# CUAI/Edge-Proposal-Sets

Measured on AMD Instinct MI355X. Metric: candidate edges scored/sec on ogbl-ppa (ppa-like synthetic): Adamic-Adar over the FULL 2-hop non-edge candidate set + top-4M selection, higher is better.
Workload: dtype int64

## Files before the change

### edge-proposal-sets_amd/csrc/scan_pieces.hip

```cpp
#include "eps_common.h"
#include "scan_common.h"
#include <string.h>

#define SP_EMPTY 0u
#define SP_MAXP (SP_M + 1)
#define SP_UBITS 8192
#define SP_SB 4
#define SP_PACKED_X8 8u
#define SP_MODE_RATIO 2270u
#define SP_MODE_RATIO_WIDE 8000u
#define SP_BATCH 8
#define SP_EM 128
#define SP_G 1

typedef int sp_v4i __attribute__((ext_vector_type(4)));

struct sp_params {
    const int64_t *rowptr;
    const int32_t *col;
    const int32_t *revpos;
    const uint32_t *fx32;
    const float *val;
    const float *node_w;
    float up;
// ... 6 lines not shown
    uint32_t col_bytes;
    int32_t table_bits;
    uint32_t piece_paths;
    const uint32_t *ssum;
    const uint32_t *smax;
    uint32_t packed_paths;
    int32_t packed_dmax;
    const uint32_t *pptr;
    const uint4 *plan;
    uint32_t mode_ratio;
    int32_t shift;
    float scale;
    unsigned int *next_col;
    eps_survivors *out;
    unsigned int *status;
    const uint4 *colrec;
    const uint32_t *rowrec;
    uint32_t wide_paths;
    int32_t wide_rows;
    uint32_t sketch;
    uint32_t batch_from;
    const uint4 *pack;
    const uint2 *heads;
};

__device__ __forceinline__ void sp_barrier() { asm volatile("s_waitcnt lgkmcnt(0)\n\ts_barrier" ::: "memory"); }

__device__ __forceinline__ int sp_wave_incl_scan(int x)
{
    x += __builtin_amdgcn_update_dpp(0, x, 0x111, 0xF, 0xF, false);
    x += __builtin_amdgcn_update_dpp(0, x, 0x112, 0xF, 0xF, false);
    x += __builtin_amdgcn_update_dpp(0, x, 0x114, 0xF, 0xF, false);
    x += __builtin_amdgcn_update_dpp(0, x, 0x118, 0xF, 0xF, false);
    x += __builtin_amdgcn_update_dpp(0, x, 0x142, 0xA, 0xF, false);
    x += __builtin_amdgcn_update_dpp(0, x, 0x143, 0xC, 0xF, false);
    return x;
}

__device__ __forceinline__ uint32_t sp_wave_sum(uint32_t x)
{
    return (uint32_t)__builtin_amdgcn_readlane(sp_wave_incl_scan((int)x), 63);
}

typedef float sp_v4f __attribute__((ext_vector_type(4)));
typedef short sp_v2s __attribute__((ext_vector_type(2)));

__device__ __forceinline__ uint32_t sp_mix(uint32_t x) { return x * 0x9E3779B1u; }
__device__ __forceinline__ uint32_t sp_mix2(uint32_t x) { return x * 0x85EBCA6Bu; }

struct sp_unit {
    sp_v4i u4;
    sp_v4f a4;
    uint32_t fx;
    int nvalid;
};

template <class Emit>
__device__ __forceinline__ int sp_plan_column(const sp_params &p, int32_t v, int32_t dv, int lane, int32_t my_bound, uint32_t pwk,
                                              int32_t nbk, uint32_t direct_ids, Emit emit)
{
    const uint32_t ek = (uint32_t)sp_wave_incl_scan((int)pwk) - pwk;
    const bool pk_on = p.ssum != nullptr;
    const uint32_t sv = pk_on ? p.ssum[v] - (p.heads ? (p.heads[v].y < p.ssum[v] ? p.heads[v].y : p.ssum[v]) : 0u) : 0u;
    const uint32_t smk = pk_on ? p.smax[lane <= SP_M ? lane : SP_M] : 0u;
    const int kv = __popcll(__ballot(lane >= 1 && lane < SP_M && my_bound <= v - 1));
    const int32_t hi_k = my_bound < v ? my_bound : v;
    int np = 0, k0 = 0;
    while (k0 <= kv) {
        const int32_t lo = __builtin_amdgcn_readlane(my_bound, k0);
        const uint32_t e0 = (uint32_t)__builtin_amdgcn_readlane((int)ek, k0);
        const bool in = lane > k0 && lane <= kv + 1;
// ... 66 lines not shown
template <int T, bool HV, bool FULL, bool PACK, bool SK = false>
__global__ __launch_bounds__(T, 4) void scan_piece_kernel(sp_params p)
{
    extern __shared__ __attribute__((aligned(16))) uint32_t lds[];
    const int slots = 1 << p.table_bits;
    uint32_t *tkey = lds;
    uint32_t *tval = lds + slots;
    uint4 *r_desc = (uint4 *)(lds + 2 * slots);
    uint32_t *ubits = lds + ((2 * slots + 4 * (T + 1) + 3) & ~3);
    uint16_t *wrank = (uint16_t *)(ubits + SP_UBITS / 32);
    __shared__ unsigned long long s_alloc;
    __shared__ int s_rbase;
    __shared__ int32_t s_pk0[SP_MAXP], s_pk1[SP_MAXP];
    __shared__ int32_t s_plo[SP_MAXP], s_phi[SP_MAXP];
    __shared__ uint32_t s_pinfo[SP_MAXP];
    __shared__ uint32_t s_pq[SP_MAXP];
    __shared__ int32_t s_pna[SP_MAXP], s_pnb[SP_MAXP];
    __shared__ int s_np;
    __shared__ unsigned int s_ticket;
    __shared__ unsigned int s_out_cur, s_out_end;
    __shared__ unsigned int s_fill_lo, s_fill_hi;
    __shared__ unsigned int s_hot;
    __shared__ uint32_t s_em[SP_EM];

    const int tid = threadIdx.x, lane = tid & 63;
    const int wib = __builtin_amdgcn_readfirstlane(tid >> 6);
    const uint32_t out_cap = p.out->capacity;
    int64_t *__restrict__ out_key = p.out->key;
    float *__restrict__ out_val = p.out->val;
    const uint32_t *__restrict__ rowptr_lo = (const uint32_t *)p.rowptr;
    const __amdgpu_buffer_rsrc_t col_rs = __builtin_amdgcn_make_buffer_rsrc((void *)p.col, 0, p.col_bytes, 0x00020000);
    const __amdgpu_buffer_rsrc_t val_rs = __builtin_amdgcn_make_buffer_rsrc((void *)(HV ? (const void *)p.val : (const void *)p.col), 0,
                                                                            p.col_bytes, 0x00020000);
    const uint32_t thr32 = sp_bar_units(p.out->threshold, p.shift);
    const uint32_t direct_ids = 2u * (uint32_t)slots;
    const bool no_bar = !FULL && thr32 <= 1u;
    const bool raw_sums = FULL || p.heads != nullptr;
    const uint32_t chunk = no_bar && direct_ids > 8192u ? direct_ids : 8192u;
    const int32_t my_bound = p.bounds[lane <= SP_M ? lane : SP_M];

    for (int i = tid; i < 2 * slots; i += T) lds[i] = 0u;
    for (int i = tid; i < SP_UBITS / 32; i += T) ubits[i] = 0u;
    for (int i = tid; i < SP_EM; i += T) s_em[i] = 0u;
    if (tid == 0) {
        s_out_cur = 0u;
        s_out_end = 0u;
        s_fill_lo = 0u;
        s_fill_hi = 0u;
        s_alloc = 0ull;
    }
    bool sketch_seen = false;
    unsigned long long n_cand = 0;
    uint32_t new_keys = 0u;
    const unsigned int ncol = (unsigned int)p.n_columns;
    const unsigned int batch_from = p.batch_from;
    auto first_of = [&](unsigned int tk) { return tk < batch_from ? tk : batch_from + (tk - batch_from) * SP_BATCH; };
    unsigned int t = blockIdx.x < batch_from ? blockIdx.x : first_of(blockIdx.x);
    unsigned int t_end = t + (blockIdx.x < batch_from ? 1u : SP_BATCH);
    sp_barrier();

    while (t < ncol) {
        const bool last_of_ticket = t + 1u >= t_end || t + 1u >= ncol;
        unsigned int t_next = 0;
        if (tid == 0 && last_of_ticket) t_next = gridDim.x + atomicAdd(p.next_col, 1u);
        int32_t v, dv;
        uint32_t vb;
        uint4 cra = make_uint4(0u, 0u, 0u, 0u), crb = make_uint4(0u, 0u, 0u, 0u);
        if (FULL || p.colrec) {
            cra = p.colrec[2 * (size_t)t];
            crb = p.colrec[2 * (size_t)t + 1];
            v = (int32_t)cra.x;
            vb = cra.y;
            dv = (int32_t)cra.z;
        } else {
            v = p.columns[t];
            vb = rowptr_lo[2 * (size_t)v];
            dv = (int32_t)(rowptr_lo[2 * (size_t)v + 2] - vb);
        }
        const int32_t *__restrict__ vcol = p.col + vb;
        const int32_t *__restrict__ vrev = p.revpos + vb;
        const int rounds = (dv + T - 1) / T;
        const bool single = rounds == 1;
        uint32_t xv = 0u, thr_v = thr32;
        bool bad_head = false;
        if (FULL || p.heads) {
            const uint2 hd = (FULL || p.colrec) ? make_uint2(cra.w, crb.x) : p.heads[v];
            xv = hd.x;
            if (thr32 < SP_FLAG) {
                bad_head = hd.y >= thr32;
                thr_v = thr32 - hd.y;
            }
            if (bad_head && tid == 0) atomicOr(p.status, 4u);
            if ((FULL || p.ssum) && thr32 < SP_FLAG && ((FULL || p.colrec) ? crb.y : p.ssum[v]) < thr32) bad_head = true;
        }
        if (dv > 0 && v > 0 && !bad_head) {
            uint32_t my_w = 0, my_rev = 0, my_base = 0, my_fx = 0;
            uint32_t cut_first = 0u;
            if (PACK && single && tid < dv) {
                const uint4 pa = p.pack[2 * ((size_t)vb + (size_t)tid)];
                my_w = pa.x;
                my_base = pa.y;
                my_fx = pa.z;
                my_rev = pa.w & 0xFFFFu;
                cut_first = pa.w >> 16;
            }
            if (!PACK && single && tid < dv) {
                my_w = (uint32_t)vcol[tid];
                my_rev = (uint32_t)vrev[tid];
            }
            if (!PACK && single && tid < dv) {
                my_base = (FULL || p.rowrec) ? p.rowrec[(size_t)my_w * 32 + 16] : rowptr_lo[2 * (size_t)my_w];
                my_fx = HV ? __builtin_bit_cast(uint32_t, (p.val[vb + tid] * p.node_w[my_w]) * p.up)
                           : ((FULL || p.rowrec) ? p.rowrec[(size_t)my_w * 32 + 17] : p.fx32[my_w]);
            }
            if (!FULL && wib == 0 && !p.plan) {
                const uint32_t pwk = lane < SP_M ? p.wpaths[(size_t)v * SP_M + lane] : 0u;
                const int32_t nbk = lane >= 1 && lane <= SP_M ? (int32_t)p.cuts[(size_t)v * SP_M + lane - 1] : 0;
                const int np = sp_plan_column(p, v, dv, lane, my_bound, pwk, nbk, direct_ids,
                                              [&](int i, int k0, int k1, int32_t lo, int32_t hi, uint32_t info, uint32_t pq, int32_t na, int32_t nb) {
                                                  if (lane == 0) {
                                                      s_pk0[i] = k0;
                                                      s_pk1[i] = k1;
                                                      s_plo[i] = lo;
                                                      s_phi[i] = hi;
                                                      s_pinfo[i] = info;
                                                      s_pq[i] = pq;
                                                      s_pna[i] = na;
                                                      s_pnb[i] = nb;
                                                  }
                                              });
                if (lane == 0) s_np = np;
            } else if (FULL || p.plan) {
                const uint32_t pb = (FULL || p.colrec) ? crb.z : p.pptr[v];
                const int np = (FULL || p.colrec) ? (int)crb.w : (int)(p.pptr[v + 1] - pb);
                if (tid < np) {
                    const uint4 rec = p.plan[pb + (uint32_t)tid];
                    const int k1 = (int)((rec.y >> 8) & 0xFFu);
                    const int32_t bk = p.bounds[k1];
                    s_pinfo[tid] = rec.x;
                    s_pk0[tid] = (int)(rec.y & 0xFFu);
                    s_pk1[tid] = k1;
                    s_pq[tid] = rec.y >> 16;
                    s_pna[tid] = (int32_t)(rec.z & 0xFFFFu);
                    s_pnb[tid] = (int32_t)(rec.z >> 16);
                    s_plo[tid] = (int32_t)rec.w;
                    s_phi[tid] = bk < v ? bk : v;
                }
                if (tid == 0) s_np = np;
            }
            sp_barrier();
            const int np = s_np;
            uint32_t cut_ahead = 0u, seg_from = 0u;
            const uint16_t *__restrict__ cut_tab = (FULL || p.rowrec) ? (const uint16_t *)p.rowrec : p.cuts;
            const size_t cut_ld = (FULL || p.rowrec) ? 64u : (size_t)SP_M;
// ... 34 lines not shown
                const uint32_t mask = (1u << bits) - 1u;
                const uint32_t span = (uint32_t)(hi_id - lo_id);
                const uint32_t scan_slots = d16 ? (span + 1u) >> 1 : direct ? span : (1u << bits);
                const uint32_t cand_max = direct ? span : (1u << bits);
                if (tid == 0) {
                    s_hot = 0u;
                    uint32_t need = ppaths < cand_max ? ppaths : cand_max;
                    if (!no_bar && need > 1024u) need = 1024u;
                    if (need > chunk) need = chunk;
                    const uint32_t left = s_out_cur < s_out_end ? s_out_end - s_out_cur : 0u;
                    if (left < need) {
                        s_fill_lo = s_out_cur < out_cap ? s_out_cur : out_cap;
                        s_fill_hi = left ? (s_out_end < out_cap ? s_out_end : out_cap) : s_fill_lo;
                        const unsigned long long b64 = atomicAdd(&p.out->count, (unsigned long long)chunk);
                        const uint32_t b = b64 < (unsigned long long)out_cap ? (uint32_t)b64 : out_cap;
                        s_out_cur = b;
                        s_out_end = b + chunk;
                    }
                }
                uint32_t seg_a = 0u, seg_len = 0u;
                if (single && tid < dv) {
                    const uint32_t b = cut_ahead < my_rev ? cut_ahead : my_rev;
                    seg_a = seg_from;
                    seg_len = (uint32_t)tid < xv ? 0u : b - seg_from;
                    seg_from = b;
                    if (pi + 1 < np)
                        cut_ahead = PACK && pi + 1 <= 8 ? pack16[((size_t)vb + (size_t)tid) * 16 + 7 + (pi + 1)]
                                                        : cut_tab[(size_t)my_w * cut_ld + s_pk1[pi + 1] - 1];
                }
                auto emit = [&](uint32_t u, uint32_t sum) {
                    uint32_t pos = atomicAdd(&s_out_cur, 1u);
                    if (pos >= s_out_end) {
                        const unsigned long long q = atomicAdd(&p.out->count, 1ull);
                        pos = q < (unsigned long long)out_cap ? (uint32_t)q : out_cap;
                    }
                    if (pos < out_cap) {
                        out_key[pos] = ((int64_t)v << 32) | (int64_t)u;
                        out_val[pos] = raw_sums ? __builtin_bit_cast(float, sum) : (float)sum * p.scale;
                    }
                };
                for (uint32_t part = 0; part < parts; ++part) {
                    for (int j = sketch ? nb : single ? tid : na + tid; j < nb; j += T) {
                        const uint32_t u = single ? my_w : (uint32_t)vcol[j];
                        if (j >= na && (int32_t)u >= lo_id && (int32_t)u < hi_id) {
                            if (d16) {
                                const uint32_t o = u - (uint32_t)lo_id;
                                atomicOr(&lds[o >> 1], 0x8000u << ((o & 1u) << 4));
                            } else if (direct) {
                                lds[u - (uint32_t)lo_id] = SP_FLAG;
                            } else if (packed) {
                                const uint32_t mix = sp_mix(u);
                                uint32_t h = mix >> (32 - bits);
                                const uint32_t st = ((mix >> 7) | 1u) & mask;
                                const uint32_t word = ((u - (uint32_t)lo_id) << pk_sb) | pk_flag;
                                for (uint32_t tries = 0; tries <= mask; ++tries) {
                                    if (atomicCAS(&lds[h], 0u, word) == 0u) break;
                                    h = (h + st) & mask;
                                }
                            } else {
                                const uint32_t mix = sp_mix(u);
                                if ((mix & (parts - 1u)) == part) {
                                    uint32_t h = mix >> (32 - bits);
                                    const uint32_t st = ((mix >> 7) | 1u) & mask;
// ... 91 lines not shown
                            for (int q = 0; q < SP_G; ++q) {
                                const int s = (int)ulo + (it0 + q) * T + tid;
                                const uint4 rd = r_desc[lo[q]];
                                const uint32_t us = rd.w, rl = rd.y, rs = rd.x;
                                f[q].fx = rd.z;
                                const bool in = s < (int)uhi;
                                const int off = (s - (int)us) * 4;
                                int left = (int)rl - off;
                                left = in ? left : 0;
                                f[q].nvalid = left < 0 ? 0 : (left > 4 ? 4 : left);
                                const uint32_t at = in ? rs + (uint32_t)off : (p.col_bytes >> 2);
                                f[q].u4 = __builtin_amdgcn_raw_buffer_load_b128(col_rs, (int)(at * 4u), 0, 0);
                                if (HV) f[q].a4 = __builtin_bit_cast(sp_v4f, __builtin_amdgcn_raw_buffer_load_b128(val_rs, (int)(at * 4u), 0, 0));
                            }
                        };
                        auto path_fx = [&](const sp_unit &f, int e) -> uint32_t {
                            if (!HV) return f.fx;
                            return (uint32_t)__builtin_ceilf(f.a4[e] * __builtin_bit_cast(float, f.fx)) + 1u;
                        };
                        auto consume_group = [&](const sp_unit (&f)[SP_G]) {
                            if (sketch) {
                                const uint32_t half = 1u << (bits - 1);
#pragma unroll
                                for (int q = 0; q < SP_G; ++q)
#pragma unroll
                                    for (int e = 0; e < 4; ++e)
                                        if (e < f[q].nvalid) {
                                            const uint32_t id = (uint32_t)f[q].u4[e];
                                            atomicAdd(&lds[sp_mix(id) >> (33 - bits)], f[q].fx);
                                            atomicAdd(&lds[half + (sp_mix2(id) >> (33 - bits))], f[q].fx);
                                        }
                            } else if (d16) {
#pragma unroll
                                for (int q = 0; q < SP_G; ++q)
#pragma unroll
                                    for (int e = 0; e < 4; ++e)
                                        if (e < f[q].nvalid) {
                                            const uint32_t o = (uint32_t)(f[q].u4[e] - lo_id);
                                            atomicAdd(&lds[o >> 1], f[q].fx << ((o & 1u) << 4));
                                        }
                            } else if (direct) {
#pragma unroll
                                for (int q = 0; q < SP_G; ++q)
#pragma unroll
                                    for (int e = 0; e < 4; ++e)
                                        if (e < f[q].nvalid) atomicAdd(&lds[(uint32_t)(f[q].u4[e] - lo_id)], path_fx(f[q], e));
                            } else if (packed) {
                                constexpr int E = 4 * SP_G;
                                uint32_t lid[E], h[E], mixv[E], old[E];
                                uint32_t pend = 0u;
#pragma unroll
                                for (int q = 0; q < SP_G; ++q) pend |= ((1u << f[q].nvalid) - 1u) << (4 * q);
#pragma unroll
                                for (int i = 0; i < E; ++i) {
// ... 126 lines not shown
                                        have = false;
                                        pend = 0u;
                                    }
                                }
                            }
                        };
                        {
                            const int n_iter = (int)(uhi - ulo + T - 1) / T;
                            sp_unit fa[SP_G], fb[SP_G];
                            fetch_group(0, fa);
                            if (n_iter <= SP_G) {
                                consume_group(fa);
                            } else {
                                for (int it0 = 0; it0 < n_iter; it0 += 2 * SP_G) {
                                    fetch_group(it0 + SP_G, fb);
                                    consume_group(fa);
                                    fetch_group(it0 + 2 * SP_G, fa);
                                    consume_group(fb);
                                }
                            }
                        }
                        if (sketch) {
                            if (tid == 0 && !sketch_seen) atomicOr(p.status, 16u);
                            sketch_seen = true;
                            sp_barrier();
                            const uint32_t half = 1u << (bits - 1);
                            {
                                uint32_t mx = 0u;
                                for (uint32_t i = 4u * (uint32_t)tid; i < half; i += 4u * T) {
                                    const uint4 a4 = *(const uint4 *)(lds + i);
                                    const uint32_t m01 = a4.x > a4.y ? a4.x : a4.y, m23 = a4.z > a4.w ? a4.z : a4.w;
                                    const uint32_t m = m01 > m23 ? m01 : m23;
                                    mx = m > mx ? m : mx;
                                }
                                if (__ballot(mx >= thr_v) && lane == 0) s_hot = 1u;
                            }
                            sp_barrier();
                            if (s_hot) {
                            const int n_iter = (int)(uhi - ulo + T - 1) / T;
                            auto report = [&](uint32_t u, uint32_t est) {
                                int a = na, b = nb;
                                while (a < b) {
                                    const int mid = (a + b) >> 1;
                                    if (vcol[mid] < (int32_t)u) a = mid + 1; else b = mid;
                                }
                                if (a < nb && vcol[a] == (int32_t)u) return;
                                const uint32_t em_mask = (p.sketch >> 1 ? p.sketch >> 1 : (uint32_t)SP_EM) - 1u;
                                uint32_t h = (sp_mix(u) >> 9) & em_mask;
                                for (uint32_t tries = 0; tries <= em_mask; ++tries) {
                                    const uint32_t old = atomicCAS(&s_em[h], 0u, u + 1u);
                                    if (old == 0u) {
                                        emit(u, est);
                                        return;
                                    }
                                    if (old == u + 1u) return;
                                    h = (h + 1u) & em_mask;
                                }
                                atomicOr(p.status, 8u);
                            };
                            auto look = [&](const sp_unit (&f)[SP_G]) {
                                uint32_t est[4 * SP_G];
#pragma unroll
                                for (int i = 0; i < 4 * SP_G; ++i) {
                                    const uint32_t id = (uint32_t)f[i >> 2].u4[i & 3];
                                    const uint32_t ea = lds[sp_mix(id) >> (33 - bits)], eb = lds[half + (sp_mix2(id) >> (33 - bits))];
                                    est[i] = ea < eb ? ea : eb;
                                }
#pragma unroll
                                for (int i = 0; i < 4 * SP_G; ++i)
                                    if ((i & 3) < f[i >> 2].nvalid && est[i] >= thr_v) report((uint32_t)f[i >> 2].u4[i & 3], est[i]);
                            };
                            sp_unit fa[SP_G], fb[SP_G];
                            fetch_group(0, fa);
                            if (n_iter <= SP_G) {
                                look(fa);
                            } else {
                                for (int it0 = 0; it0 < n_iter; it0 += 2 * SP_G) {
                                    fetch_group(it0 + SP_G, fb);
                                    look(fa);
                                    fetch_group(it0 + 2 * SP_G, fa);
                                    look(fb);
                                }
                            }
                            }
                        }
                            if (uhi < (uint32_t)total) sp_barrier();
                        }
                        sp_barrier();
                        for (int i = tid; i < SP_UBITS / 32; i += T) ubits[i] = 0u;
                        if (tid == 0) {
                            s_alloc = 0ull;
                            s_fill_hi = 0u;
                        }
// ... 97 lines not shown
                            for (int b = 0; b < SP_SB; ++b) {
                                const uint32_t i = i0 + 4u * T * b + 4u * tid;
                                const int sv[4] = {(int)s4[b].x, (int)s4[b].y, (int)s4[b].z, (int)s4[b].w};
                                const int m01 = sv[0] > sv[1] ? sv[0] : sv[1], m23 = sv[2] > sv[3] ? sv[2] : sv[3];
                                if ((m01 > m23 ? m01 : m23) >= thr_s) {
#pragma unroll
                                    for (int e = 0; e < 4; ++e)
                                        if (sv[e] >= thr_s) emit(tkey[i + e] - 1u, (uint32_t)sv[e]);
                                }
                                if (i < scan_slots) {
                                    *(uint4 *)(tkey + i) = make_uint4(0u, 0u, 0u, 0u);
                                    *(uint4 *)(tval + i) = make_uint4(0u, 0u, 0u, 0u);
                                }
                            }
                        }
                    }
                    n_cand += (unsigned long long)cnt_here + (unsigned long long)new_keys;
                    new_keys = 0u;
                    sp_barrier();
                }
            }
        }
        if (!last_of_ticket) {
            ++t;
            sp_barrier();
            continue;
        }
        if (tid == 0) s_ticket = t_next;
        sp_barrier();
        const unsigned int tk = s_ticket;
        sp_barrier();
        t = first_of(tk);
        t_end = t + (tk < batch_from ? 1u : SP_BATCH);
    }
    {
        const uint32_t f0 = s_out_cur < out_cap ? s_out_cur : out_cap, f1 = s_out_end < out_cap ? s_out_end : out_cap;
        for (uint32_t i = f0 + (uint32_t)tid; i < f1; i += T) {
            out_key[i] = -1;
            out_val[i] = -__builtin_inff();
        }
    }
    {
        unsigned long long x = n_cand;
#pragma unroll
        for (int d = 32; d >= 1; d >>= 1) x += __shfl_xor(x, d);
        if (lane == 0 && x) atomicAdd(&p.out->n_candidates, x);
    }
// ... 616 lines not shown
    EPS_REQUIRE((ssum_or_null == nullptr) == (smax_or_null == nullptr), "eps_scan_screen: ssum and smax come together");
    EPS_REQUIRE(!heads_or_null || plan_or_null, "eps_scan_screen: a head table comes with the plan table built for it");
    return sp_launch(rowptr, col, nullptr, revpos, fx32, nullptr, cuts, wpaths, ssum_or_null, smax_or_null, pptr_or_null,
                     plan_or_null, heads_or_null, rowrec_or_null, pack_or_null, bounds, n_nodes, nnz, columns, colrec_or_null, n_columns,
                     batch_from, shift, variant, out, status, stream);
}

extern "C" int eps_scan_screen_weighted(const int64_t *rowptr, const int32_t *col, const float *val, const int32_t *revpos,
                                        const float *node_w, const uint16_t *cuts, const uint32_t *wpaths,
                                        const int32_t *bounds, int64_t n_nodes, int64_t nnz, const int32_t *columns,
                                        int64_t n_columns, int32_t shift, int32_t variant, eps_survivors *out, uint32_t *status,
                                        void *stream)
{
    EPS_REQUIRE(n_columns == 0 || n_nodes == 0 || (val && node_w), "eps_scan_screen_weighted: null pointer");
    return sp_launch(rowptr, col, val, revpos, nullptr, node_w, cuts, wpaths, nullptr, nullptr, nullptr, nullptr, nullptr, nullptr, nullptr,
                     bounds, n_nodes, nnz, columns, nullptr, n_columns, n_columns, shift, variant, out, status, stream);
}

static const int sp_threads_of[3] = {512, 1024, 256}, sp_bits_of[3] = {13, 14, 12}, sp_per_cu[3] = {2, 1, 4};
#define SP_VARIANT_GEOM(v) ((v) & 0xFF)
#define SP_VARIANT_DMAX(v) ((((v) >> 8) & 0xFF) - 1)
#define SP_VARIANT_WIDE(v) (((v) >> 24) & 1)
#define SP_VARIANT_SKETCH(v) (((v) >> 16) & 0xFF)

static void sp_plan_geometry(sp_params &p, const uint16_t *cuts, const uint32_t *wpaths, const uint32_t *ssum, const uint32_t *smax,
                             const int32_t *bounds, int64_t n_nodes, int32_t shift, int32_t variant, int32_t dmax_arg)
{
    const int bits = sp_bits_of[variant];
    p.cuts = cuts;
    p.wpaths = wpaths;
    p.bounds = bounds;
    p.n_nodes = (int32_t)n_nodes;
    p.table_bits = bits;
    p.piece_paths = (1u << bits) / 2u;
    p.ssum = ssum;
    p.smax = smax;
    p.packed_paths = (SP_PACKED_X8 << bits) / 8u;
    p.packed_dmax = shift > 8 ? (shift - 8 < 24 ? shift - 8 : 24) : 0;
    if (dmax_arg >= 0 && dmax_arg < p.packed_dmax) p.packed_dmax = dmax_arg;
    p.mode_ratio = SP_MODE_RATIO;
    p.shift = shift;
}

__global__ __launch_bounds__(256) void sp_plan_kernel(sp_params p, const int64_t *__restrict__ rowptr, uint32_t direct_ids,
                                                      uint32_t *__restrict__ pcount, const uint32_t *__restrict__ pptr, uint4 *__restrict__ out,
                                                      uint32_t *__restrict__ d_used)
// ... 101 lines not shown
                       (1u << sp_bits_of[variant]) / 2u, out2);
    EPS_CHECK_LAUNCH("eps_scan_plan_rewalk");
    return EPS_OK;
}

static int sp_launch(const int64_t *rowptr, const int32_t *col, const float *val, const int32_t *revpos, const uint32_t *fx32,
                     const float *node_w, const uint16_t *cuts, const uint32_t *wpaths, const uint32_t *ssum, const uint32_t *smax,
                     const uint32_t *pptr, const uint32_t *plan, const uint32_t *heads, const uint32_t *rowrec, const uint32_t *pack,
                     const int32_t *bounds, int64_t n_nodes, int64_t nnz, const int32_t *columns, const uint32_t *colrec, int64_t n_columns, int64_t batch_from,
                     int32_t shift, int32_t variant, eps_survivors *out, uint32_t *status, void *stream)
{
    EPS_REQUIRE(n_nodes >= 0 && n_columns >= 0 && nnz >= 0, "eps_scan_screen: negative size");
    EPS_REQUIRE(status, "eps_scan_screen: null pointer");
    hipStream_t s = (hipStream_t)stream;
    if (hipMemsetAsync(status, 0, sizeof(uint32_t), s) != hipSuccess) {
        eps_set_error("eps_scan_screen: cannot clear the status word");
        return EPS_ELAUNCH;
    }
    if (n_columns == 0 || n_nodes == 0) return EPS_OK;
    EPS_REQUIRE(rowptr && col && revpos && cuts && wpaths && bounds && columns && out, "eps_scan_screen: null pointer");
    EPS_REQUIRE(nnz < (1ll << 30), "eps_scan_screen: col[] is addressed with 32-bit byte offsets (nnz < 2^30)");
    EPS_REQUIRE(n_nodes < (1ll << 31) && n_columns < (1ll << 31), "eps_scan_screen: too many nodes / columns");
    const uint32_t sketch_arg = (uint32_t)SP_VARIANT_SKETCH(variant);
    EPS_REQUIRE(!SP_VARIANT_WIDE(variant) || ((sketch_arg & 1u) && plan && !val && SP_VARIANT_GEOM(variant) == 2),
                "eps_scan_screen: a plan with wide packed pieces (variant bit 24) is for sketch launches (bit 16) of the 256-thread geometry");
    const int32_t dmax_arg = SP_VARIANT_DMAX(variant);
    variant = SP_VARIANT_GEOM(variant);
    EPS_REQUIRE(shift >= 0 && shift <= 40 && variant >= 0 && variant <= 2, "eps_scan_screen: bad shift / variant");
    EPS_REQUIRE(((uintptr_t)cuts & 15) == 0, "eps_scan_screen: cuts must be 16-byte aligned");
    EPS_REQUIRE(((uintptr_t)colrec & 15) == 0 && ((uintptr_t)rowrec & 127) == 0, "eps_scan_screen: misaligned column / row records");
    EPS_REQUIRE(!colrec || plan, "eps_scan_screen: column records come with the plan table they were built from");
    EPS_REQUIRE((pptr == nullptr) == (plan == nullptr) && ((uintptr_t)plan & 15) == 0, "eps_scan_screen: pptr and plan come together, 16-byte aligned");
    const int T = sp_threads_of[variant], bits = sp_bits_of[variant];
    unsigned int *counter = nullptr;
    const int rc = eps_take_counter(&counter, s, "eps_scan_screen");
    if (rc) return rc;
    sp_params p;
    memset(&p, 0, sizeof p);
    p.rowptr = rowptr;
    p.col = col;
    p.revpos = revpos;
    p.fx32 = fx32;
    p.val = val;
    p.node_w = node_w;
    p.up = ldexpf(1.0f, shift) * (1.0f + ldexpf(1.0f, -20));
    sp_plan_geometry(p, cuts, wpaths, ssum, smax, bounds, n_nodes, shift, variant, dmax_arg);
// ... 8 lines not shown
    p.batch_from = batch_from < 0 || batch_from > n_columns ? (uint32_t)n_columns : (uint32_t)batch_from;
    p.sketch = val || !(sketch_arg & 1u) ? 0u : sketch_arg;
    p.col_bytes = (uint32_t)(nnz * 4);
    p.scale = ldexpf(1.0f, -shift);
    p.next_col = counter;
    p.out = out;
    p.status = status;
    int64_t blocks = (int64_t)eps_num_cus() * sp_per_cu[variant];
    if (blocks > n_columns) blocks = n_columns;
    const size_t lds = ((size_t)(2 << bits) + 4 * (size_t)(T + 1) + 8) * 4 + (SP_UBITS / 32) * 6 + 32;
    void (*kern)(sp_params) =
        val ? (variant == 0 ? scan_piece_kernel<512, true, false, false> : variant == 1 ? scan_piece_kernel<1024, true, false, false>
                                                                                       : scan_piece_kernel<256, true, false, false>)
            : (variant == 0 ? scan_piece_kernel<512, false, false, false> : variant == 1 ? scan_piece_kernel<1024, false, false, false>
                                                                                         : scan_piece_kernel<256, false, false, false>);
    const bool full = !val && variant == 2 && plan && colrec && rowrec && heads && ssum;
    EPS_REQUIRE(!pack || full, "eps_scan_screen: the column pack serves the main launch only (variant 2, plan, records, heads, sum bounds)");
    if (full) kern = pack ? scan_piece_kernel<256, false, true, true> : scan_piece_kernel<256, false, true, false>;
    if (p.sketch && variant == 2)
        kern = full ? (pack ? scan_piece_kernel<256, false, true, true, true> : scan_piece_kernel<256, false, true, false, true>)
                    : scan_piece_kernel<256, false, false, false, true>;
    else
        p.sketch = 0u;
    if (hipFuncSetAttribute((const void *)kern, hipFuncAttributeMaxDynamicSharedMemorySize, (int)lds) != hipSuccess) {
        eps_set_error("eps_scan_screen: cannot reserve %zu bytes of LDS", lds);
        return EPS_ELAUNCH;
    }
    hipLaunchKernelGGL(kern, dim3((unsigned)blocks), dim3(T), lds, s, p);
    EPS_CHECK_LAUNCH("eps_scan_screen");
    return EPS_OK;
}

__global__ void scan_pieces_warm_kernel() {}
extern "C" void eps_warm_scan_pieces(void *stream) { hipLaunchKernelGGL(scan_pieces_warm_kernel, dim3(1), dim3(1), 0, (hipStream_t)stream); }
```

### edge-proposal-sets_amd/ops.py

```python
from __future__ import annotations

import ctypes
from typing import Optional, Sequence, Tuple

import torch

from . import _lib

W_AA, W_RA = 0, 1


_EMPTY = {}


def _ptr(t: Optional[torch.Tensor]):
    if t is None:
        return None
    if t.numel() == 0 and t.is_cuda:
        key = (t.device.type, t.device.index)
        if key not in _EMPTY:
            _EMPTY[key] = torch.zeros(8, dtype=torch.int64, device=t.device)
        return ctypes.c_void_p(_EMPTY[key].data_ptr())
    return ctypes.c_void_p(t.data_ptr())

# ... 733 lines not shown
def scan_bounds(rowptr, n_nodes: int) -> torch.Tensor:
    dev = _need_gpu(rowptr)
    _chk(rowptr, torch.int64, "rowptr")
    out = torch.empty(scan_windows() + 1, dtype=torch.int32, device=dev)
    with torch.cuda.device(dev):
        _lib.check(_lib.load().eps_scan_bounds(_ptr(rowptr), n_nodes, _ptr(out), _stream(dev)), "eps_scan_bounds")
    return out


def scan_row_sums(rowptr, col, fx32: torch.Tensor, bounds: torch.Tensor, n_nodes: int):
    dev = _need_gpu(rowptr, col, fx32, bounds)
    _chk(rowptr, torch.int64, "rowptr"); _chk(col, torch.int32, "col"); _chk(fx32, torch.int32, "fx32"); _chk(bounds, torch.int32, "bounds")
    m = scan_windows()
    buf = torch.empty(n_nodes + 2 * m + 2, dtype=torch.int32, device=dev)
    ssum, smax, min_fx, ws = buf[:n_nodes], buf[n_nodes:n_nodes + m + 1], buf[n_nodes + m + 1:n_nodes + m + 2], buf[n_nodes + m + 2:]
    with torch.cuda.device(dev):
        _lib.check(_lib.load().eps_scan_row_sums(_ptr(rowptr), _ptr(col), _ptr(fx32), _ptr(bounds), n_nodes, _ptr(ssum), _ptr(smax),
                                                 _ptr(min_fx), _ptr(ws), _stream(dev)), "eps_scan_row_sums")
    return ssum, smax, min_fx


SCAN_WIDE = 1 << 24
SCAN_SKETCH = 1 << 16


def scan_variant_word(variant: int, dmax: Optional[int] = None) -> int:
    return int(variant) | ((min(int(dmax), 254) + 1) << 8 if dmax is not None else 0)


def scan_plan(rowptr, cuts, wpaths, ssum, smax, bounds, n_nodes: int, shift: int, variant: int, with_d: bool = False,
              heads: Optional[torch.Tensor] = None):
    dev = _need_gpu(rowptr, cuts, wpaths, ssum, smax, bounds, heads)
    _chk_heads(heads, n_nodes)
    _chk(rowptr, torch.int64, "rowptr"); _chk(cuts, torch.int16, "cuts"); _chk(wpaths, torch.int32, "wpaths")
    _chk(ssum, torch.int32, "ssum"); _chk(smax, torch.int32, "smax"); _chk(bounds, torch.int32, "bounds")
    lib = _lib.load()
    counts = torch.empty(n_nodes, dtype=torch.int32, device=dev)
    with torch.cuda.device(dev):
        _lib.check(lib.eps_scan_plan(_ptr(rowptr), _ptr(cuts), _ptr(wpaths), _ptr(ssum), _ptr(smax), _ptr(heads), _ptr(bounds), n_nodes,
                                     int(shift), int(variant), _ptr(counts), None, None, None, _stream(dev)), "eps_scan_plan")
        pptr = torch.zeros(n_nodes + 1, dtype=torch.int32, device=dev)
        if n_nodes:
            torch.cumsum(counts, 0, dtype=torch.int32, out=pptr[1:])
        n_rec = int(pptr[-1].item()) if n_nodes else 0
        recs = torch.empty((max(n_rec, 1), 4), dtype=torch.int32, device=dev)
        d_used = torch.zeros(1, dtype=torch.int32, device=dev) if with_d else None
# ... 487 lines not shown
```

### edge-proposal-sets_amd/scan.py

```python
from __future__ import annotations

from collections import namedtuple
from typing import List, Optional, Tuple

import torch

from . import ops
from .graph import CSRGraph

SAMPLE_STRIDE = 256
SAFETY = 2.0
SMALL_SET = 1 << 25
MAX_K = 1 << 30
MAX_LAUNCHES = 8
_CHUNK_SLACK = 8192 * 320
RELABEL_MIN_NODES = 100_000
ONE_PASS = True
_PIECE_SLACK = 8192 * 1024 + 65536
MAX_SCREEN_SHIFT = 30
HEADS = True
HEAD_BETA = 0.5
HEAD_KEEP = (0.3, 0.58)
HEAD_LIST = 2
HEAD_MIN_PATHS = 1 << 30
HEAD_MAX_ROWS = 1024
HEAD_CACHE = 4
DMAX_MARGIN = 5
FORCE_SHARDED = False


def _sharded(world: int) -> bool:
    return world > 1 or FORCE_SHARDED


SKETCH_PIECES = True
SKETCH_MIN_PATHS = 1.5
SKETCH_SET = 0
LAZY_PLAN = True
BATCH_MIN_COLUMNS = 1 << 16
BATCH_PATHS = 1 << 13


def scan_available(g: CSRGraph) -> bool:
    if not (scan_plausible(g) and is_symmetric(g)):
        return False
    return g.val is None or (values_symmetric(g) and screen_variant(scan_graph(g)[0]) is not None)


def scan_plausible(g: CSRGraph) -> bool:
    return bool(g.device.type == "cuda" and g.n_rows == g.n_cols and 0 < g.n_rows <= ops.filter_scan_max_nodes() and g.nnz() < 1 << 30)


def scan_usable(g: CSRGraph, node_w: torch.Tensor) -> bool:
    from . import candidates
    if not (scan_available(g) and candidates.fused_scores_fit(g, node_w)):
        return False
    if g.val is None:
        return True
    gs, perm = scan_graph(g)
# ... 379 lines not shown
                        v = variant
                        break
        g._cache["screen_variant"] = v
    return g._cache["screen_variant"]


def one_pass_available(g: CSRGraph) -> bool:
    return screen_variant(g) is not None


def _launch(g, fixw, columns, threshold, capacity, scores_only: bool = False, both: bool = False, screen=None,
            heads: Optional[HeadTables] = None, walked_capacity: int = 0, sample_key=None, sketch: bool = False) -> ops.Survivors:
    out = ops.Survivors(capacity, threshold, g.device, scores_only, both, prefill=screen is None)
    out.walked_slots = None
    if screen is not None:
        out.status = torch.empty(1, dtype=torch.int32, device=g.device)
        if not columns.numel():
            out.status.zero_()
    if columns.numel():
        if screen is not None and heads is not None:
            bounds, cuts = screen_tables(g)
            walked = ops.Survivors(walked_capacity, threshold, g.device, prefill=False)
            ops.scan_screen(g.rowptr, g.col, reverse_positions(g), screen.fx32, cuts, bounds, g.n_rows, columns, screen.shift, walked,
                            out.status, screen_variant(g) | ((ops.SCAN_SKETCH | SKETCH_SET << 17) if sketch else 0) | (ops.SCAN_WIDE if heads.wide else 0), None, None, heads.wpaths, screen.ssum, screen.smax,
                            heads.plan, heads.heads,
                            batch_from(g, columns), screen.rowrec,
                            column_records(g, screen, columns, heads.plan, heads.heads, heads.live, ("colrec", columns.data_ptr(), columns.numel())),
                            column_pack(g, screen, heads) if variant_is_main(g, screen) else None)
            ops.scan_refine(walked, heads.heads, hub_rows(g), screen.fx32, g.rowptr, g.col, g.n_rows, screen.shift, out)
            out.rec[4:5].copy_(walked.rec[4:5])
            out.walked_slots = walked.rec[1:2]
        elif screen is not None:
            bounds, cuts = screen_tables(g)
            if sample_key is not None and screen.val is None and screen._plan is None and screen._plan_build is not None:
                wp, plan = sample_window_paths(g, columns, sample_key), None
            else:
                wp, plan = window_paths(g), screen.plan
            ops.scan_screen(g.rowptr, g.col, reverse_positions(g), screen.fx32, cuts, bounds, g.n_rows, columns, screen.shift, out,
                            out.status, screen.vword if screen.vword is not None and screen.val is None else screen_variant(g),
                            screen.val, screen.node_w, wp, screen.ssum, screen.smax, plan,
                            None, batch_from(g, columns), screen.rowrec)
        else:
            ops.filter_scan(g.rowptr, g.col, reverse_positions(g), fixw, g.n_rows, columns, out, max_degree(g), window_splits(g))
    return out


def variant_is_main(g: CSRGraph, screen: Screen) -> bool:
# ... 240 lines not shown


def _capacity(slots_wanted: int, slack: Optional[int] = None) -> int:
    cap = int(slots_wanted) + (_CHUNK_SLACK if slack is None else slack)
    if cap > ops.SURVIVOR_SLOTS_MAX:
        raise ops._lib.EpsError(f"scan_topk: a survivor list of {cap} slots exceeds the {ops.SURVIVOR_SLOTS_MAX} a launch can "
                                "address (slots are 32-bit positions); use the block-streaming filter path for this set")
    return cap


Verdict = namedtuple("Verdict", "action launches drop_heads head_trouble head_stale")


def _verdict(table, capacity: int, walked_cap: int, head_budget: Optional[int], shift: Optional[int], screened: bool,
             rescore_all: bool, k2: int, bar_set: bool, launches: int, head_trouble: int = 0, head_stale: int = 0) -> Verdict:
    def again(action: str, failing: str, drop_heads: bool = False) -> Verdict:
        n = launches - 1
        if n + 2 > MAX_LAUNCHES:
            raise ops._lib.EpsError(f"scan_topk: {failing} kept failing")
        return Verdict(action, n, drop_heads, head_trouble, head_stale)

    if any(t[4] & 8 for t in table):
        return again("sketch off", "launches with sketch pieces")
    if any(t[4] & ~(4 | 16) for t in table):
        raise ops._lib.EpsError("scan_topk: eps_scan_screen reported a full hash table (status %s)" % [t[4] for t in table])
    drop_heads = False
    if head_budget is not None:
        bar_units = _f32_from_bits(table[0][7]) * 2.0 ** shift
        overflow = any(t[6] > walked_cap for t in table)
        stale = any(t[4] & 4 for t in table) or head_budget > HEAD_KEEP[1] * bar_units
        drop_heads = overflow or stale or not HEAD_KEEP[0] * bar_units <= head_budget <= HEAD_KEEP[1] * bar_units
        if overflow or stale:
            head_trouble, head_stale = head_trouble + overflow, head_stale + (not overflow)
            action = "heads off" if head_trouble >= 2 or head_stale >= 3 else "grow walked list" if overflow else "rebuild heads"
            return again(action, "launches with skipped heads", drop_heads)
    slot_overflow = any(t[0] > capacity for t in table)
    cut_is_inf = (table[0][3] & 0xFFFFFFFF) == 0xFF800000
    if screened and not rescore_all and not slot_overflow:
        cut_f = float("-inf") if cut_is_inf else _f32_from_bits(table[0][3])
        if any(cut_f < _f32_from_bits(t[5]) for t in table):
            return again("rescore all", "the re-scoring pre-filter", drop_heads)
    if slot_overflow:
        return Verdict("rescan wider" if cut_is_inf else "rescan below cut", launches, drop_heads, head_trouble, head_stale)
    n_cand, n_sel = sum(t[1] for t in table), sum(t[2] for t in table)
    if bar_set and n_sel < (k2 if head_budget is not None else min(k2, n_cand)):
        return Verdict("drop bar" if launches > 3 else "lower bar", launches, drop_heads, head_trouble, head_stale)
    return Verdict("done", launches, drop_heads, head_trouble, head_stale)
# ... 143 lines not shown
                                                   None if rows_on == "shards" else rows_on)
        elif rows_on is None or rows_on == rank or rows_on == "shards":
            keys, vals = ops.select_rows(keys.contiguous(), vals.contiguous(), k, bits, perm)
        else:
            keys = vals = None
        if rows_on == "shards" and keys is not None:
            n_rows = keys.numel()
            lo_r, hi_r = rank * n_rows // world, (rank + 1) * n_rows // world
            shard = (lo_r, n_rows)
            keys, vals = keys[lo_r:hi_r], vals[lo_r:hi_r]
    if keys is None:
        return None, None, shard
    return torch.stack([keys & 0xFFFFFFFF, keys >> 32]), vals, shard


def _step_stats(stats: dict, g: CSRGraph, screen: Optional[Screen], fixw, table, ht: Optional[HeadTables], capacity: int,
                launches: int, sketch_void: int, n_rescored, shard, bar, rank: int, world: int) -> None:
    n_cand, n_sel = sum(t[1] for t in table), sum(t[2] for t in table)
    if ht is None and world == 1:
        g._cache.setdefault("n_candidates", n_cand)
    n_all = 2 * n_cand if ht is None else 2 * candidate_count(g, screen, fixw, rank, world) if stats.get("count", True) else None
    stats.update(candidates=n_all, touched=2 * n_cand, launches=launches, survivors=2 * n_sel, heads=ht is not None, shard=shard,
                 sketch=any(t[4] & 16 for t in table), sketch_void=sketch_void,
                 head_budget=None if ht is None else ht.budget * 2.0 ** -screen.shift,
                 walked_slots=sum(t[6] for t in table) if ht is not None else None, rescored=n_rescored,
                 survivor_slots=sum(min(t[0], capacity) for t in table), bar=bar)


def scan_topk(g: CSRGraph, node_w: torch.Tensor, k: int, rank: int = 0, world: int = 1, stats: Optional[dict] = None,
              relabel: bool = False, rows_on: Optional[int] = None):
    if relabel and scan_plausible(g):
        scan_graph(g, build=True)
    if not scan_available(g):
        raise ops._lib.EpsError("scan_topk: graph not supported by eps_filter_scan (see scan_available)")
    k = int(k)
    if not 0 < k <= MAX_K:
        raise ops._lib.EpsError(f"scan_topk: k = {k} outside (0, {MAX_K}] (longer lists: the block-streaming filter path)")
    from . import candidates
    if not candidates.fused_scores_fit(g, node_w):
        raise ops._lib.EpsError(f"scan_topk: score bound {candidates.fused_score_bound(g, node_w):.3e} of this graph / weight "
                                "table leaves the 2^-40 fixed-point range of the scan (use the pair kernels)")
    g0 = g
    g, perm = scan_graph(g0, relabel)
    fixw = _scan_weights(g0, g, perm, node_w) if g.val is None else None
    mine = shard_columns(g, rank, world)
    total_half = total_half_paths(g)
# ... 94 lines not shown
```

Before: 1275 billion.

## Batch several light sketch columns into one block pass with salted sketch keys

In the batched tail of the sketch scan, a block now gathers up to eight consecutive light columns (single-round, one plan piece) and processes them together as a single combined column. Each column gets a 3-bit salt in the high bits of fx, which keeps the shared count-min sketch hash keys and the emit-dedup keys separate per column. Reports resolve back to the source column for the non-edge check, threshold and output key. The aim is to stop spending one full block iteration (barriers, LDS clears, sketch sweep) on each tiny column. In exchange it adds per-batch planning in wave 0, sharing one LDS sketch across columns (more collisions), and a new status bit.

```diff
diff --git a/edge-proposal-sets_amd/csrc/scan_pieces.hip b/edge-proposal-sets_amd/csrc/scan_pieces.hip
--- a/edge-proposal-sets_amd/csrc/scan_pieces.hip
+++ b/edge-proposal-sets_amd/csrc/scan_pieces.hip
@@ -52,6 +52,7 @@
     uint32_t batch_from;
     const uint4 *pack;
     const uint2 *heads;
+    uint32_t light_paths;
 };
 
 __device__ __forceinline__ void sp_barrier() { asm volatile("s_waitcnt lgkmcnt(0)\n\ts_barrier" ::: "memory"); }
@@ -77,6 +78,8 @@
 
 __device__ __forceinline__ uint32_t sp_mix(uint32_t x) { return x * 0x9E3779B1u; }
 __device__ __forceinline__ uint32_t sp_mix2(uint32_t x) { return x * 0x85EBCA6Bu; }
+#define SP_FXMASK 0x1FFFFFFFu
+__device__ __forceinline__ uint32_t sp_salt(uint32_t fx) { return (fx >> 29) * 0x27D4EB2Fu; }
 
 struct sp_unit {
     sp_v4i u4;
@@ -189,6 +192,9 @@
     __shared__ unsigned int s_fill_lo, s_fill_hi;
     __shared__ unsigned int s_hot;
     __shared__ uint32_t s_em[SP_EM];
+    __shared__ uint4 s_tka[SP_BATCH], s_tkb[SP_BATCH], s_ba[SP_BATCH];
+    __shared__ uint2 s_bb[SP_BATCH];
+    __shared__ uint32_t s_bn, s_bskip, s_bdv, s_bpaths, s_bkeys, s_bthr;
 
     const int tid = threadIdx.x, lane = tid & 63;
     const int wib = __builtin_amdgcn_readfirstlane(tid >> 6);
@@ -216,7 +222,7 @@
         s_fill_hi = 0u;
         s_alloc = 0ull;
     }
-    bool sketch_seen = false;
+    bool sketch_seen = false, light_seen = false;
     unsigned long long n_cand = 0;
     uint32_t new_keys = 0u;
     const unsigned int ncol = (unsigned int)p.n_columns;
@@ -227,13 +233,82 @@
     sp_barrier();
 
     while (t < ncol) {
-        const bool last_of_ticket = t + 1u >= t_end || t + 1u >= ncol;
+        uint32_t nbat = 0u, nskip = 1u;
+        if (FULL && PACK && SK && p.light_paths && t >= batch_from && thr32 < SP_FLAG) {
+            const unsigned int t0 = t_end - SP_BATCH;
+            if (wib == 0) {
+                const unsigned int tj = t0 + (unsigned int)lane;
+                uint4 a = make_uint4(0u, 0u, 0u, 0u), b = make_uint4(2u, 0u, 0u, 0u);
+                if (t == t0) {
+                    if (lane < SP_BATCH && tj < ncol) {
+                        a = p.colrec[2 * (size_t)tj];
+                        const uint4 rb = p.colrec[2 * (size_t)tj + 1];
+                        const bool bad = rb.x >= thr32;
+                        const bool idle = !bad && (a.z == 0u || a.x == 0u || rb.y < thr32);
+                        const bool one = !bad && !idle && rb.w == 1u && a.z <= (uint32_t)T;
+                        const uint4 pl = one ? p.plan[rb.z] : make_uint4(0u, 0u, 0u, 0u);
+                        b = make_uint4(idle ? 0u : one && (pl.x >> 30) == 1u ? 1u : 2u, thr32 - rb.x, pl.x & 0x3FFFFFFFu, pl.z);
+                    }
+                    if (lane < SP_BATCH) {
+                        s_tka[lane] = a;
+                        s_tkb[lane] = b;
+                    }
+                } else if (lane < SP_BATCH) {
+                    a = s_tka[lane];
+                    b = s_tkb[lane];
+                }
+                const int s = (int)(t - t0);
+                const bool live = lane >= s && lane < SP_BATCH && tj < ncol && b.x <= 1u;
+                const int end0 = __ffsll((long long)__ballot(lane >= s && !live)) - 1;
+                const bool q = live && lane < end0 && b.x == 1u;
+                const uint32_t qdv = q ? a.z : 0u, qp = q ? b.z : 0u;
+                const uint32_t inc_dv = (uint32_t)sp_wave_incl_scan((int)qdv), inc_p = (uint32_t)sp_wave_incl_scan((int)qp);
+                const unsigned long long over = __ballot(q && (inc_dv > (uint32_t)T || inc_p > p.light_paths));
+                const int end = over ? __ffsll((long long)over) - 1 : end0;
+                const unsigned long long mem = __ballot(q && lane < end);
+                const int n = __popcll(mem);
+                if (n >= 2) {
+                    const int c = __popcll(mem & ((1ull << lane) - 1ull));
+                    if ((mem >> lane) & 1ull) {
+                        s_ba[c] = make_uint4(a.x, a.y, inc_dv - a.z, a.w);
+                        s_bb[c] = make_uint2(b.y, b.w);
+                    }
+                    const uint32_t m = (mem >> lane) & 1ull;
+                    const uint32_t keys = sp_wave_sum(m ? b.z + (b.w >> 16) - (b.w & 0xFFFFu) : 0u);
+                    const uint32_t dv_all = sp_wave_sum(qdv * m), p_all = sp_wave_sum(qp * m);
+                    uint32_t tmin = SP_FLAG;
+#pragma unroll
+                    for (int i = 0; i < SP_BATCH; ++i) {
+                        const uint32_t x = (uint32_t)__builtin_amdgcn_readlane((int)(m ? b.y : SP_FLAG), i);
+                        tmin = x < tmin ? x : tmin;
+                    }
+                    if (lane == 0) {
+                        s_bn = (uint32_t)n;
+                        s_bskip = (uint32_t)(end - s);
+                        s_bdv = dv_all;
+                        s_bpaths = p_all;
+                        s_bkeys = keys;
+                        s_bthr = tmin;
+                    }
+                } else if (lane == 0) {
+                    s_bn = 0u;
+                }
+            }
+            sp_barrier();
+            nbat = s_bn;
+            nskip = nbat ? s_bskip : 1u;
+        }
+        const bool last_of_ticket = t + nskip >= t_end || t + nskip >= ncol;
         unsigned int t_next = 0;
         if (tid == 0 && last_of_ticket) t_next = gridDim.x + atomicAdd(p.next_col, 1u);
         int32_t v, dv;
         uint32_t vb;
         uint4 cra = make_uint4(0u, 0u, 0u, 0u), crb = make_uint4(0u, 0u, 0u, 0u);
-        if (FULL || p.colrec) {
+        if (nbat) {
+            v = 1;
+            vb = 0u;
+            dv = (int32_t)s_bdv;
+        } else if (FULL || p.colrec) {
             cra = p.colrec[2 * (size_t)t];
             crb = p.colrec[2 * (size_t)t + 1];
             v = (int32_t)cra.x;
@@ -250,7 +325,9 @@
         const bool single = rounds == 1;
         uint32_t xv = 0u, thr_v = thr32;
         bool bad_head = false;
-        if (FULL || p.heads) {
+        if (nbat) {
+            thr_v = s_bthr;
+        } else if (FULL || p.heads) {
             const uint2 hd = (FULL || p.colrec) ? make_uint2(cra.w, crb.x) : p.heads[v];
             xv = hd.x;
             if (thr32 < SP_FLAG) {
@@ -264,16 +341,27 @@
             uint32_t my_w = 0, my_rev = 0, my_base = 0, my_fx = 0;
             uint32_t cut_first = 0u;
             if (PACK && single && tid < dv) {
-                const uint4 pa = p.pack[2 * ((size_t)vb + (size_t)tid)];
+                uint32_t at = vb + (uint32_t)tid, cb = 0u;
+                bool head_row = (uint32_t)tid < xv;
+                if (nbat) {
+                    uint32_t c = 0u;
+#pragma unroll
+                    for (int i = 1; i < SP_BATCH; ++i) c += (uint32_t)i < nbat && (uint32_t)tid >= s_ba[i].z ? 1u : 0u;
+                    const uint4 ba = s_ba[c];
+                    at = ba.y + ((uint32_t)tid - ba.z);
+                    head_row = (uint32_t)tid - ba.z < ba.w;
+                    cb = c << 29;
+                }
+                const uint4 pa = p.pack[2 * (size_t)at];
                 my_w = pa.x;
                 my_base = pa.y;
-                my_fx = pa.z;
-                my_rev = pa.w & 0xFFFFu;
+                my_fx = pa.z | cb;
+                my_rev = head_row ? 0u : pa.w & 0xFFFFu;
                 cut_first = pa.w >> 16;
             }
             if (!PACK && single && tid < dv) {
                 my_w = (uint32_t)vcol[tid];
-                my_rev = (uint32_t)vrev[tid];
+                my_rev = (uint32_t)tid < xv ? 0u : (uint32_t)vrev[tid];
             }
             if (!PACK && single && tid < dv) {
                 my_base = (FULL || p.rowrec) ? p.rowrec[(size_t)my_w * 32 + 16] : rowptr_lo[2 * (size_t)my_w];
@@ -297,6 +385,18 @@
                                                   }
                                               });
                 if (lane == 0) s_np = np;
+            } else if (nbat) {
+                if (tid == 0) {
+                    s_pinfo[0] = s_bpaths | 0x40000000u;
+                    s_pk0[0] = 0;
+                    s_pk1[0] = 1;
+                    s_pq[0] = 0u;
+                    s_pna[0] = 0;
+                    s_pnb[0] = (int32_t)(s_bkeys - s_bpaths);
+                    s_plo[0] = 0;
+                    s_phi[0] = 0;
+                    s_np = 1;
+                }
             } else if (FULL || p.plan) {
                 const uint32_t pb = (FULL || p.colrec) ? crb.z : p.pptr[v];
                 const int np = (FULL || p.colrec) ? (int)crb.w : (int)(p.pptr[v + 1] - pb);
@@ -377,23 +477,24 @@
                 if (single && tid < dv) {
                     const uint32_t b = cut_ahead < my_rev ? cut_ahead : my_rev;
                     seg_a = seg_from;
-                    seg_len = (uint32_t)tid < xv ? 0u : b - seg_from;
+                    seg_len = b - seg_from;
                     seg_from = b;
                     if (pi + 1 < np)
                         cut_ahead = PACK && pi + 1 <= 8 ? pack16[((size_t)vb + (size_t)tid) * 16 + 7 + (pi + 1)]
                                                         : cut_tab[(size_t)my_w * cut_ld + s_pk1[pi + 1] - 1];
                 }
-                auto emit = [&](uint32_t u, uint32_t sum) {
+                auto emit_to = [&](int32_t vv, uint32_t u, uint32_t sum) {
                     uint32_t pos = atomicAdd(&s_out_cur, 1u);
                     if (pos >= s_out_end) {
                         const unsigned long long q = atomicAdd(&p.out->count, 1ull);
                         pos = q < (unsigned long long)out_cap ? (uint32_t)q : out_cap;
                     }
                     if (pos < out_cap) {
-                        out_key[pos] = ((int64_t)v << 32) | (int64_t)u;
+                        out_key[pos] = ((int64_t)vv << 32) | (int64_t)u;
                         out_val[pos] = raw_sums ? __builtin_bit_cast(float, sum) : (float)sum * p.scale;
                     }
                 };
+                auto emit = [&](uint32_t u, uint32_t sum) { emit_to(v, u, sum); };
                 for (uint32_t part = 0; part < parts; ++part) {
                     for (int j = sketch ? nb : single ? tid : na + tid; j < nb; j += T) {
                         const uint32_t u = single ? my_w : (uint32_t)vcol[j];
@@ -531,14 +632,16 @@
                             if (sketch) {
                                 const uint32_t half = 1u << (bits - 1);
 #pragma unroll
-                                for (int q = 0; q < SP_G; ++q)
+                                for (int q = 0; q < SP_G; ++q) {
+                                    const uint32_t salt = sp_salt(f[q].fx), w = f[q].fx & SP_FXMASK;
 #pragma unroll
                                     for (int e = 0; e < 4; ++e)
                                         if (e < f[q].nvalid) {
-                                            const uint32_t id = (uint32_t)f[q].u4[e];
-                                            atomicAdd(&lds[sp_mix(id) >> (33 - bits)], f[q].fx);
-                                            atomicAdd(&lds[half + (sp_mix2(id) >> (33 - bits))], f[q].fx);
+                                            const uint32_t id = (uint32_t)f[q].u4[e] ^ salt;
+                                            atomicAdd(&lds[sp_mix(id) >> (33 - bits)], w);
+                                            atomicAdd(&lds[half + (sp_mix2(id) >> (33 - bits))], w);
                                         }
+                                }
                             } else if (d16) {
 #pragma unroll
                                 for (int q = 0; q < SP_G; ++q)
@@ -711,7 +814,9 @@
                         }
                         if (sketch) {
                             if (tid == 0 && !sketch_seen) atomicOr(p.status, 16u);
+                            if (tid == 0 && nbat && !light_seen) atomicOr(p.status, 64u);
                             sketch_seen = true;
+                            light_seen = light_seen || nbat;
                             sp_barrier();
                             const uint32_t half = 1u << (bits - 1);
                             {
@@ -727,22 +832,34 @@
                             sp_barrier();
                             if (s_hot) {
                             const int n_iter = (int)(uhi - ulo + T - 1) / T;
-                            auto report = [&](uint32_t u, uint32_t est) {
+                            auto report = [&](uint32_t u, uint32_t est, uint32_t c) {
                                 int a = na, b = nb;
+                                const int32_t *__restrict__ vc = vcol;
+                                int32_t vv = v;
+                                if (nbat) {
+                                    const uint4 ba = s_ba[c];
+                                    const uint32_t nanb = s_bb[c].y;
+                                    a = (int)(nanb & 0xFFFFu);
+                                    b = (int)(nanb >> 16);
+                                    vc = p.col + ba.y;
+                                    vv = (int32_t)ba.x;
+                                }
+                                const int e_nb = b;
                                 while (a < b) {
                                     const int mid = (a + b) >> 1;
-                                    if (vcol[mid] < (int32_t)u) a = mid + 1; else b = mid;
-                                }
-                                if (a < nb && vcol[a] == (int32_t)u) return;
+                                    if (vc[mid] < (int32_t)u) a = mid + 1; else b = mid;
+                                }
+                                if (a < e_nb && vc[a] == (int32_t)u) return;
                                 const uint32_t em_mask = (p.sketch >> 1 ? p.sketch >> 1 : (uint32_t)SP_EM) - 1u;
-                                uint32_t h = (sp_mix(u) >> 9) & em_mask;
+                                const uint32_t key = (c << 29 | u) + 1u;
+                                uint32_t h = (sp_mix(key - 1u) >> 9) & em_mask;
                                 for (uint32_t tries = 0; tries <= em_mask; ++tries) {
-                                    const uint32_t old = atomicCAS(&s_em[h], 0u, u + 1u);
+                                    const uint32_t old = atomicCAS(&s_em[h], 0u, key);
                                     if (old == 0u) {
-                                        emit(u, est);
+                                        emit_to(vv, u, est);
                                         return;
                                     }
-                                    if (old == u + 1u) return;
+                                    if (old == key) return;
                                     h = (h + 1u) & em_mask;
                                 }
                                 atomicOr(p.status, 8u);
@@ -751,13 +868,18 @@
                                 uint32_t est[4 * SP_G];
 #pragma unroll
                                 for (int i = 0; i < 4 * SP_G; ++i) {
-                                    const uint32_t id = (uint32_t)f[i >> 2].u4[i & 3];
+                                    const uint32_t id = (uint32_t)f[i >> 2].u4[i & 3] ^ sp_salt(f[i >> 2].fx);
                                     const uint32_t ea = lds[sp_mix(id) >> (33 - bits)], eb = lds[half + (sp_mix2(id) >> (33 - bits))];
                                     est[i] = ea < eb ? ea : eb;
                                 }
 #pragma unroll
-                                for (int i = 0; i < 4 * SP_G; ++i)
-                                    if ((i & 3) < f[i >> 2].nvalid && est[i] >= thr_v) report((uint32_t)f[i >> 2].u4[i & 3], est[i]);
+                                for (int q = 0; q < SP_G; ++q) {
+                                    const uint32_t c = f[q].fx >> 29;
+                                    const uint32_t thr_c = nbat ? s_bb[c].x : thr_v;
+#pragma unroll
+                                    for (int e = 0; e < 4; ++e)
+                                        if (e < f[q].nvalid && est[4 * q + e] >= thr_c) report((uint32_t)f[q].u4[e], est[4 * q + e], c);
+                                }
                             };
                             sp_unit fa[SP_G], fb[SP_G];
                             fetch_group(0, fa);
@@ -901,7 +1023,7 @@
             }
         }
         if (!last_of_ticket) {
-            ++t;
+            t += nskip;
             sp_barrier();
             continue;
         }
@@ -1564,6 +1686,7 @@
 #define SP_VARIANT_DMAX(v) ((((v) >> 8) & 0xFF) - 1)
 #define SP_VARIANT_WIDE(v) (((v) >> 24) & 1)
 #define SP_VARIANT_SKETCH(v) (((v) >> 16) & 0xFF)
+#define SP_VARIANT_LIGHT(v) (((v) >> 25) & 1)
 
 static void sp_plan_geometry(sp_params &p, const uint16_t *cuts, const uint32_t *wpaths, const uint32_t *ssum, const uint32_t *smax,
                              const int32_t *bounds, int64_t n_nodes, int32_t shift, int32_t variant, int32_t dmax_arg)
@@ -1711,6 +1834,7 @@
     EPS_REQUIRE(nnz < (1ll << 30), "eps_scan_screen: col[] is addressed with 32-bit byte offsets (nnz < 2^30)");
     EPS_REQUIRE(n_nodes < (1ll << 31) && n_columns < (1ll << 31), "eps_scan_screen: too many nodes / columns");
     const uint32_t sketch_arg = (uint32_t)SP_VARIANT_SKETCH(variant);
+    const bool light_arg = SP_VARIANT_LIGHT(variant) != 0;
     EPS_REQUIRE(!SP_VARIANT_WIDE(variant) || ((sketch_arg & 1u) && plan && !val && SP_VARIANT_GEOM(variant) == 2),
                 "eps_scan_screen: a plan with wide packed pieces (variant bit 24) is for sketch launches (bit 16) of the 256-thread geometry");
     const int32_t dmax_arg = SP_VARIANT_DMAX(variant);
@@ -1765,6 +1889,8 @@
                     : scan_piece_kernel<256, false, false, false, true>;
     else
         p.sketch = 0u;
+    if (light_arg && p.sketch && full && pack && n_nodes < (1ll << 29))
+        p.light_paths = (2u << bits) < (uint32_t)SP_UBITS ? (2u << bits) : (uint32_t)SP_UBITS;
     if (hipFuncSetAttribute((const void *)kern, hipFuncAttributeMaxDynamicSharedMemorySize, (int)lds) != hipSuccess) {
         eps_set_error("eps_scan_screen: cannot reserve %zu bytes of LDS", lds);
         return EPS_ELAUNCH;
diff --git a/edge-proposal-sets_amd/ops.py b/edge-proposal-sets_amd/ops.py
--- a/edge-proposal-sets_amd/ops.py
+++ b/edge-proposal-sets_amd/ops.py
@@ -779,6 +779,7 @@
 
 SCAN_WIDE = 1 << 24
 SCAN_SKETCH = 1 << 16
+SCAN_LIGHT = 1 << 25
 
 
 def scan_variant_word(variant: int, dmax: Optional[int] = None) -> int:
diff --git a/edge-proposal-sets_amd/scan.py b/edge-proposal-sets_amd/scan.py
--- a/edge-proposal-sets_amd/scan.py
+++ b/edge-proposal-sets_amd/scan.py
@@ -35,6 +35,7 @@
 
 SKETCH_PIECES = True
 SKETCH_MIN_PATHS = 1.5
+LIGHT_BATCH = True
 SKETCH_SET = 0
 LAZY_PLAN = True
 BATCH_MIN_COLUMNS = 1 << 16
@@ -460,7 +461,7 @@
             bounds, cuts = screen_tables(g)
             walked = ops.Survivors(walked_capacity, threshold, g.device, prefill=False)
             ops.scan_screen(g.rowptr, g.col, reverse_positions(g), screen.fx32, cuts, bounds, g.n_rows, columns, screen.shift, walked,
-                            out.status, screen_variant(g) | ((ops.SCAN_SKETCH | SKETCH_SET << 17) if sketch else 0) | (ops.SCAN_WIDE if heads.wide else 0), None, None, heads.wpaths, screen.ssum, screen.smax,
+                            out.status, screen_variant(g) | ((ops.SCAN_SKETCH | SKETCH_SET << 17 | (ops.SCAN_LIGHT if LIGHT_BATCH else 0)) if sketch else 0) | (ops.SCAN_WIDE if heads.wide else 0), None, None, heads.wpaths, screen.ssum, screen.smax,
                             heads.plan, heads.heads,
                             batch_from(g, columns), screen.rowrec,
                             column_records(g, screen, columns, heads.plan, heads.heads, heads.live, ("colrec", columns.data_ptr(), columns.numel())),
@@ -747,7 +748,7 @@
 
     if any(t[4] & 8 for t in table):
         return again("sketch off", "launches with sketch pieces")
-    if any(t[4] & ~(4 | 16) for t in table):
+    if any(t[4] & ~(4 | 16 | 64) for t in table):
         raise ops._lib.EpsError("scan_topk: eps_scan_screen reported a full hash table (status %s)" % [t[4] for t in table])
     drop_heads = False
     if head_budget is not None:
@@ -937,6 +938,7 @@
     n_all = 2 * n_cand if ht is None else 2 * candidate_count(g, screen, fixw, rank, world) if stats.get("count", True) else None
     stats.update(candidates=n_all, touched=2 * n_cand, launches=launches, survivors=2 * n_sel, heads=ht is not None, shard=shard,
                  sketch=any(t[4] & 16 for t in table), sketch_void=sketch_void,
+                 light_batches=any(t[4] & 64 for t in table),
                  head_budget=None if ht is None else ht.budget * 2.0 ** -screen.shift,
                  walked_slots=sum(t[6] for t in table) if ht is not None else None, rescored=n_rescored,
                  survivor_slots=sum(min(t[0], capacity) for t in table), bar=bar)
```

After: 1281 billion, median of 6. No clear change (+0.5%).
